# PaddlePaddle/MetaGym

Hardware: NVIDIA H100
Metric: env-steps/sec (quadrotor 6-DoF, 65k envs) (higher is better)
Workload: dtype f32

## Files before the change

metagym_b200/csrc/quad.cu:

```cuda
#include <math.h>
#include <stdlib.h>
#include <string.h>
#include <new>
#include <vector>

#include "mgb_common.cuh"
#include "quad_lanes.cuh"

namespace {

constexpr int kThreads = 64;
constexpr int kMaxObs = 19;

struct QuadConst {
    float h;
    float k1phi;
    float k1;
    float inv_phi;
    float hjm;
    float hk;
    float mm;
    float ct0, ct1, ct2;
    float vmin, vmax;
    float A[4], B[4];
    float px[4], py[4], pz[4];
    float Df[3], Dm[3];
    float cg[3];
    float hI[9];
    float gm;
    float c_hm;
    float c_h2m;
    float fail_r2, fail_v2, fail_w2;
    float dt, healthy, z_off;
    float init_v[3], init_w[3], noise_v, noise_w;
    int nt, task, substeps, obs_dim;
    int rk4_steps;
    float rk4_h;
    float inv_jm, inv_m;
    float Iinv[9];
    int simple;
};

struct QuadArgs {
    float4 *planes;
    int64_t n_pad;
    int64_t n;
    int64_t env_base;
    const float *act;
    float *obs;
    float *rew;
    uint8_t *done;
    int32_t *fail;
    float *final_obs;
    const float *targets;
    const int32_t *sat;
    int map_rows, map_cols, x_off, y_off;
    const int32_t *env2task;
    uint64_t seed;
    int auto_reset;
    int per_cta;
    int T;
    uint64_t act_seed;
    uint32_t t_base;
    float *act_out;
    MgbMirrors mir;
};

template <class T> struct VState {
    T p[3], v[3], om[3], w[4], R[9];
    int ct[Lanes<T>::N], ep[Lanes<T>::N];
};
using QState = VState<float>;

constexpr int kTileEnvs = 128;
constexpr int kPlanes = 6;

__device__ __forceinline__ float4 *tile_base(const QuadArgs &a, int64_t e)
{
    return a.planes + (e / kTileEnvs) * (kPlanes * kTileEnvs) + (e % kTileEnvs);
}

__device__ __forceinline__ void unpack_state(const float4 q[kPlanes], QState &s)
{
    s.p[0] = q[0].x; s.p[1] = q[0].y; s.p[2] = q[0].z; s.v[0] = q[0].w;
    s.v[1] = q[1].x; s.v[2] = q[1].y; s.om[0] = q[1].z; s.om[1] = q[1].w;
    s.om[2] = q[2].x; s.w[0] = q[2].y; s.w[1] = q[2].z; s.w[2] = q[2].w;
    s.w[3] = q[3].x; s.R[0] = q[3].y; s.R[1] = q[3].z; s.R[2] = q[3].w;
    s.R[3] = q[4].x; s.R[4] = q[4].y; s.R[5] = q[4].z; s.R[6] = q[4].w;
    s.R[7] = q[5].x; s.R[8] = q[5].y; s.ct[0] = __float_as_int(q[5].z); s.ep[0] = __float_as_int(q[5].w);
}
__device__ __forceinline__ void pack_state(const QState &s, float4 q[kPlanes])
{
    q[0] = make_float4(s.p[0], s.p[1], s.p[2], s.v[0]);
    q[1] = make_float4(s.v[1], s.v[2], s.om[0], s.om[1]);
    q[2] = make_float4(s.om[2], s.w[0], s.w[1], s.w[2]);
    q[3] = make_float4(s.w[3], s.R[0], s.R[1], s.R[2]);
    q[4] = make_float4(s.R[3], s.R[4], s.R[5], s.R[6]);
    q[5] = make_float4(s.R[7], s.R[8], __int_as_float(s.ct[0]), __int_as_float(s.ep[0]));
}

__device__ __forceinline__ void load_state(const QuadArgs &a, int64_t e, QState &s)
{
    const float4 *b = tile_base(a, e);
    float4 q[kPlanes];
#pragma unroll
    for (int k = 0; k < kPlanes; ++k) q[k] = b[k * kTileEnvs];
    unpack_state(q, s);
}

__device__ __forceinline__ void store_state(const QuadArgs &a, int64_t e, const QState &s)
{
    float4 *b = tile_base(a, e);
    float4 q[kPlanes];
    pack_state(s, q);
#pragma unroll
    for (int k = 0; k < kPlanes; ++k) b[k * kTileEnvs] = q[k];
}

template <class T> __device__ __forceinline__ void get_lane_state(const VState<T> &s, int h, QState &o);
template <class T> __device__ __forceinline__ void set_lane_state(VState<T> &s, int h, const QState &o);

__device__ __forceinline__ void load_state2(const QuadArgs &a, int64_t e, VState<f2> &s)
{
    QState s0, s1;
    load_state(a, e, s0);
    load_state(a, e + 1, s1);
    set_lane_state(s, 0, s0);
    set_lane_state(s, 1, s1);
}
__device__ __forceinline__ void store_state2(const QuadArgs &a, int64_t e, const VState<f2> &s)
{
    QState s0, s1;
    get_lane_state(s, 0, s0);
    get_lane_state(s, 1, s1);
    store_state(a, e, s0);
    store_state(a, e + 1, s1);
}

template <class T> __device__ __forceinline__ void get_lane_state(const VState<T> &s, int h, QState &o)
{
#pragma unroll
    for (int k = 0; k < 3; ++k) { o.p[k] = lane(s.p[k], h); o.v[k] = lane(s.v[k], h); o.om[k] = lane(s.om[k], h); }
#pragma unroll
    for (int k = 0; k < 4; ++k) o.w[k] = lane(s.w[k], h);
#pragma unroll
    for (int k = 0; k < 9; ++k) o.R[k] = lane(s.R[k], h);
    o.ct[0] = s.ct[h];
    o.ep[0] = s.ep[h];
}
template <class T> __device__ __forceinline__ void set_lane_state(VState<T> &s, int h, const QState &o)
{
#pragma unroll
    for (int k = 0; k < 3; ++k) { set_lane(s.p[k], h, o.p[k]); set_lane(s.v[k], h, o.v[k]); set_lane(s.om[k], h, o.om[k]); }
#pragma unroll
    for (int k = 0; k < 4; ++k) set_lane(s.w[k], h, o.w[k]);
#pragma unroll
    for (int k = 0; k < 9; ++k) set_lane(s.R[k], h, o.R[k]);
    s.ct[h] = o.ct[0];
    s.ep[h] = o.ep[0];
}

template <class T> __device__ __forceinline__ T dot3(T a0, T b0, T a1, T b1, T a2, T b2)
{
    return vfma(a2, b2, vfma(a1, b1, vmul(a0, b0)));
// ... 356 lines not shown
    for (int k = 0; k < 9; ++k) set_lane(s.R[k], h, (k % 4 == 0) ? 1.f : 0.f);
}

__device__ __forceinline__ void philox_reset_draws(uint64_t seed, int64_t genv, int ep, double u[12])
{
    const uint2 key = make_uint2((uint32_t)seed, (uint32_t)(seed >> 32));
#pragma unroll
    for (int j = 0; j < 3; ++j) {
        const uint4 r = mgb_philox4x32_10(
            make_uint4((uint32_t)genv, (uint32_t)((uint64_t)genv >> 32), (uint32_t)ep, MGB_STREAM_RESET + j), key);
        u[4 * j + 0] = (double)mgb_u01(r.x);
        u[4 * j + 1] = (double)mgb_u01(r.y);
        u[4 * j + 2] = (double)mgb_u01(r.z);
        u[4 * j + 3] = (double)mgb_u01(r.w);
    }
}

template <class T> struct TargetRows {
    T cur[3];
    T nxt[3];
};
template <class T>
__device__ __forceinline__ void prefetch_targets(const QuadConst &c, const float *trow, int ct, int h, TargetRows<T> &tr)
{
    const int t = ct < c.nt - 1 ? ct : c.nt - 1;
    const float *g = trow + 3 * (ct - 1), *q = trow + 3 * t;
    set_lane(tr.cur[0], h, __ldg(g)); set_lane(tr.cur[1], h, __ldg(g + 1)); set_lane(tr.cur[2], h, __ldg(g + 2));
    set_lane(tr.nxt[0], h, __ldg(q)); set_lane(tr.nxt[1], h, __ldg(q + 1)); set_lane(tr.nxt[2], h, __ldg(q + 2));
}

__device__ __forceinline__ int slice_bound(double v, int len)
{
    long long x = v < -2.0e9 ? -2000000000LL : (v > 2.0e9 ? 2000000000LL : (long long)v);
    if (x < 0) { x += len; if (x < 0) x = 0; }
    if (x > len) x = len;
    return (int)x;
}

__device__ __forceinline__ bool map_collision(const QuadArgs &a, float x_old, float y_old, float z_old, float x_new,
                                              float y_new, float z_new)
{
    const double xo = (double)x_old + a.x_off, xn = (double)x_new + a.x_off;
    const double yo = (double)y_old + a.y_off, yn = (double)y_new + a.y_off;
    const double x_min = floor(fmin(xo, xn)), x_max = ceil(fmax(xo, xn));
    const double y_min = floor(fmin(yo, yn)), y_max = ceil(fmax(yo, yn));
    const int z_lo = (int)floorf(fminf(z_old, z_new)), z_hi = (int)ceilf(fmaxf(z_old, z_new));
    const int ys = slice_bound(y_min, a.map_rows), ye = slice_bound(y_max + 1.0, a.map_rows);
    const int xs = slice_bound(x_min, a.map_cols), xe = slice_bound(x_max + 1.0, a.map_cols);
    int any = 0;
    if (ys < ye && xs < xe) {
        const int W = a.map_cols + 1;
        any = (a.sat[ye * W + xe] - a.sat[ys * W + xe] - a.sat[ye * W + xs] + a.sat[ys * W + xs]) > 0 ? 1 : 0;
    }
    return z_lo < any || z_hi < any;
}

template <class T>
__device__ __forceinline__ void observe_reset(const QuadConst &c, const QuadArgs &a, int64_t e, const VState<T> &s, int h,
                                              T *o)
{
    set_lane(o[0], h, lane(s.v[0], h)); set_lane(o[1], h, lane(s.v[1], h)); set_lane(o[2], h, lane(s.v[2], h));
    set_lane(o[3], h, 0.f); set_lane(o[4], h, 0.f); set_lane(o[5], h, 0.f);
    set_lane(o[6], h, 0.f * -9.8f); set_lane(o[7], h, 0.f * -9.8f); set_lane(o[8], h, -9.8f);
    set_lane(o[9], h, lane(s.om[0], h)); set_lane(o[10], h, lane(s.om[1], h)); set_lane(o[11], h, lane(s.om[2], h));
    set_lane(o[12], h, -0.f); set_lane(o[13], h, 0.f); set_lane(o[14], h, 0.f);
    set_lane(o[15], h, 0.f + c.z_off);
    if (c.task == MGB_TASK_VELOCITY_CONTROL) {
        const float *trow = a.targets + ((int64_t)a.env2task[e] * c.nt) * 3;
        const int t = s.ct[h] < c.nt - 1 ? s.ct[h] : c.nt - 1;
        set_lane(o[16], h, __ldg(trow + 3 * t)); set_lane(o[17], h, __ldg(trow + 3 * t + 1));
        set_lane(o[18], h, __ldg(trow + 3 * t + 2));
    }
}

template <class T>
__device__ __forceinline__ void finish_step(const QuadConst &c, const QuadArgs &a, int64_t e, VState<T> &s,
                                            const T adj[9], T id, T z_old, T x_old, T y_old, T power,
                                            const int fail[Lanes<T>::N], const TargetRows<T> &tr, T *o, T &reward,
                                            int done_flag[Lanes<T>::N], bool write_final[Lanes<T>::N])
{
    constexpr int N = Lanes<T>::N;
    T bv[3], Ri[9];
    observe(c, s, adj, id, o, bv, Ri);
    if (c.task == MGB_TASK_VELOCITY_CONTROL) {
        o[16] = tr.nxt[0]; o[17] = tr.nxt[1]; o[18] = tr.nxt[2];
    }
    reward = vneg(vmin(vmul(c.dt, power), bc<T>(c.healthy)));
    int done[N];
#pragma unroll
    for (int h = 0; h < N; ++h) done[h] = 0;
    if (c.task == MGB_TASK_VELOCITY_CONTROL) {
        const T g0 = tr.cur[0], g1 = tr.cur[1], g2 = tr.cur[2];
        T diff = bc<T>(0.f);
#pragma unroll
        for (int r = 0; r < 3; ++r) diff = vadd(diff, vabs(vsub(dot3(Ri[3 * r], g0, Ri[3 * r + 1], g1, Ri[3 * r + 2], g2), bv[r])));
        reward = vadd(reward, vmul(-0.001f, diff));
    } else {
        const T z_new = vadd(s.p[2], c.z_off);
        T bonus, vn, on;
        if (c.task == MGB_TASK_HOVERING_CONTROL) {
            vn = vsqrt(sq3(s.v));
            on = vsqrt(sq3(s.om));
        }
#pragma unroll
        for (int h = 0; h < N; ++h) {
            bool coll;
            if (a.sat) coll = map_collision(a, lane(x_old, h), lane(y_old, h), lane(z_old, h), lane(s.p[0], h),
                                            lane(s.p[1], h), lane(z_new, h));
            else coll = fminf(lane(z_old, h), lane(z_new, h)) < 0.f;
            float tr = coll ? 0.f : c.healthy;
            if (c.task == MGB_TASK_HOVERING_CONTROL) {
                tr -= lane(vn, h) + lane(on, h);
                const float zm = fabsf(0.f - lane(s.p[2], h));
                tr += zm < 0.5f ? 10.f : fmaxf(-20.f, 0.5f - zm);
            }
            set_lane(bonus, h, tr);
            if (coll) { done[h] = 1; s.ct[h] = 0; }
        }
        reward = vadd(reward, bonus);
    }
#pragma unroll
    for (int h = 0; h < N; ++h) {
        if (s.ct[h] == c.nt) { done[h] = 1; s.ct[h] = 0; }
        if (fail[h]) { done[h] = 1; s.ct[h] = 0; }
        done_flag[h] = done[h];
        write_final[h] = false;
        if (done[h] && a.auto_reset) {
            write_final[h] = true;
            s.ep[h] += 1;
            double u[12];
            philox_reset_draws(a.seed, a.env_base + e + h, s.ep[h], u);
            reset_env(c, s, h, u);
        }
    }
}

__device__ __forceinline__ void publish_tile(float *gobs, const float *tile, int64_t e0, int rows, int D)
{
    const uint32_t bytes = (uint32_t)rows * (uint32_t)D * 4u;
    float *dst = gobs + e0 * D;
    if ((bytes & 15u) == 0 && ((reinterpret_cast<uintptr_t>(dst) & 15u) == 0)) {
        mgb_fence_proxy_async();
        __syncthreads();
        if (threadIdx.x == 0) {
            mgb_bulk_store(dst, tile, bytes);
            mgb_bulk_commit();
        }
    } else {
        __syncthreads();
        for (int i = threadIdx.x; i < rows * D; i += blockDim.x) dst[i] = tile[i];
    }
}

__device__ __forceinline__ void publish_tile_mirrored(const MgbMirrors &m, float *gobs, const float *tile, int64_t e0,
                                                      int rows, int D)
{
    const uint32_t bytes = (uint32_t)rows * (uint32_t)D * 4u;
    float *dst = gobs + e0 * D;
    if ((bytes & 15u) == 0 && ((reinterpret_cast<uintptr_t>(dst) & 15u) == 0)) {
        mgb_fence_proxy_async();
        __syncthreads();
        if (threadIdx.x == 0) {
            mgb_bulk_store(dst, tile, bytes);
            mgb_mirror_bulk_store(m, dst, tile, bytes);
            mgb_bulk_commit();
        }
    } else {
        __syncthreads();
        for (int i = threadIdx.x; i < rows * D; i += blockDim.x) {
            dst[i] = tile[i];
            mgb_mirror_store(m, dst + i, tile[i]);
        }
    }
}

template <bool SIMPLE, bool EARLY, class T>
__device__ __forceinline__ void step_body(const QuadConst &c, const QuadArgs &a, int64_t e, int nact, VState<T> &s,
                                          const T V[4], float *trow, float *frow, int &final_mask)
{
    constexpr int N = Lanes<T>::N;
    const int D = c.obs_dim;
    T adj[9], id, power;
    adjugate(s.R, adj, id);
    TargetRows<T> tr;
    int ct_now[N];
#pragma unroll
    for (int h = 0; h < N; ++h) {
        s.ct[h] += 1;
        ct_now[h] = s.ct[h];
    }
    const bool vel = c.task == MGB_TASK_VELOCITY_CONTROL;
    if (EARLY && vel) {
#pragma unroll
        for (int h = 0; h < N; ++h) {
            const int64_t eh = h < nact ? e + h : e;
            prefetch_targets(c, a.targets + ((int64_t)__ldg(a.env2task + eh) * c.nt) * 3, ct_now[h], h, tr);
        }
    }
    const T z_old = vadd(s.p[2], c.z_off);
    const T x_old = s.p[0], y_old = s.p[1];
    int fail[N];
    if (N == 1 && c.rk4_steps > 0) {
        QState s1;
        get_lane_state(s, 0, s1);
        float adj1[9], id1, pw1;
        fail[0] = integrate_rk4<SIMPLE>(c, s1, make_float4(lane(V[0], 0), lane(V[1], 0), lane(V[2], 0), lane(V[3], 0)),
                                        adj1, id1, pw1);
        set_lane_state(s, 0, s1);
#pragma unroll
        for (int k = 0; k < 9; ++k) set_lane(adj[k], 0, adj1[k]);
        set_lane(id, 0, id1);
        set_lane(power, 0, pw1);
    } else {
        const bool failed = integrate<SIMPLE, T>(c, s, V, adj, id, power, fail);
        if (N > 1 && failed) {
#pragma unroll 1
            for (int h = 0; h < N; ++h) {
                QState s1;
                load_state(a, e + h, s1);
                float adj1[9], id1, pw1;
                adjugate(s1.R, adj1, id1);
                const float V1[4] = {lane(V[0], h), lane(V[1], h), lane(V[2], h), lane(V[3], h)};
                int f1[1];
                integrate<SIMPLE, float>(c, s1, V1, adj1, id1, pw1, f1);
                s1.ct[0] = s.ct[h];
                s1.ep[0] = s.ep[h];
                set_lane_state(s, h, s1);
#pragma unroll
                for (int k = 0; k < 9; ++k) set_lane(adj[k], h, adj1[k]);
                set_lane(id, h, id1);
                set_lane(power, h, pw1);
                fail[h] = f1[0];
            }
        }
    }
    if (!EARLY && vel) {
#pragma unroll
        for (int h = 0; h < N; ++h) {
            const int64_t eh = h < nact ? e + h : e;
            prefetch_targets(c, a.targets + ((int64_t)__ldg(a.env2task + eh) * c.nt) * 3, ct_now[h], h, tr);
        }
    }
    const bool state_first = N == 1 && !EARLY && vel;
    if (state_first) {
        QState s1;
        get_lane_state(s, 0, s1);
        if (s1.ct[0] == c.nt || fail[0]) s1.ct[0] = 0;
        store_state(a, e, s1);
    }
    T o[kMaxObs], reward;
    int done[N];
    bool wf[N];
    finish_step(c, a, e, s, adj, id, z_old, x_old, y_old, power, fail, tr, o, reward, done, wf);
    bool stored = false;
    if constexpr (N == 2) {
        if (nact == 2) {
            store_state2(a, e, s);
            *reinterpret_cast<float2 *>(a.rew + e) = reward.v;
            *reinterpret_cast<uchar2 *>(a.done + e) = make_uchar2((uint8_t)done[0], (uint8_t)done[1]);
            if (a.fail) *reinterpret_cast<int2 *>(a.fail + e) = make_int2(fail[0], fail[1]);
            stored = true;
        }
    }
    if (!stored) {
#pragma unroll
        for (int h = 0; h < N; ++h) {
            if (h < nact) {
                QState s1;
                get_lane_state(s, h, s1);
                if (!state_first || wf[h]) store_state(a, e + h, s1);
                a.rew[e + h] = lane(reward, h);
                a.done[e + h] = (uint8_t)done[h];
                if (a.fail) a.fail[e + h] = fail[h];
            }
        }
    }
#pragma unroll
    for (int h = 0; h < N; ++h) {
        if (h < nact) {
            float *tr_h = trow + h * D;
            if (wf[h]) {
                if (a.final_obs) {
                    float *fr_h = frow + h * D;
#pragma unroll
                    for (int k = 0; k < 16; ++k) fr_h[k] = lane(o[k], h);
                    if (D == 19) { fr_h[16] = lane(o[16], h); fr_h[17] = lane(o[17], h); fr_h[18] = lane(o[18], h); }
                    final_mask |= 1 << h;
                }
                observe_reset(c, a, e + h, s, h, o);
            }
#pragma unroll
            for (int k = 0; k < 16; ++k) tr_h[k] = lane(o[k], h);
            if (D == 19) { tr_h[16] = lane(o[16], h); tr_h[17] = lane(o[17], h); tr_h[18] = lane(o[18], h); }
        }
    }
}

__device__ __forceinline__ void publish_final(const QuadArgs &a, const float *ftile, int64_t e, int local_row, int lanes,
                                              int final_mask, int D)
{
    if (!a.final_obs) return;
    if (__syncthreads_or(final_mask)) {
        for (int h = 0; h < lanes; ++h) {
            if (final_mask & (1 << h)) {
                float *dst = a.final_obs + (e + h) * D;
                const float *frow = ftile + (local_row + h) * D;
                for (int k = 0; k < D; ++k) dst[k] = frow[k];
            }
        }
    }
}

template <bool SIMPLE>
__global__ void __launch_bounds__(kThreads) quad_step_kernel(const __grid_constant__ QuadConst c,
                                                             const __grid_constant__ QuadArgs a)
{
    __shared__ __align__(128) float tile[kThreads * kMaxObs];
    __shared__ __align__(128) float ftile[kThreads * kMaxObs];
    const int64_t e0 = (int64_t)blockIdx.x * kThreads;
    const int64_t e = e0 + threadIdx.x;
    const int rows = (int)((a.n - e0) < kThreads ? (a.n - e0) : kThreads);
    const int D = c.obs_dim;
    const bool active = e < a.n;
    int final_mask = 0;

    asm volatile("griddepcontrol.launch_dependents;");
    asm volatile("griddepcontrol.wait;" ::: "memory");

    if (active) {
        QState s;
        load_state(a, e, s);
        const float4 act = __ldg(reinterpret_cast<const float4 *>(a.act) + e);
        const float V[4] = {act.x, act.y, act.z, act.w};
        step_body<SIMPLE, false, float>(c, a, e, 1, s, V, tile + threadIdx.x * D, ftile + threadIdx.x * D, final_mask);
    }
    publish_tile(a.obs, tile, e0, rows, D);
    publish_final(a, ftile, e, threadIdx.x, 1, final_mask, D);
    if (threadIdx.x == 0) mgb_bulk_wait_read<0>();
}

template <bool SIMPLE>
__global__ void __launch_bounds__(512, 1) quad_step_wide_kernel(const __grid_constant__ QuadConst c,
                                                                const __grid_constant__ QuadArgs a)
{
    extern __shared__ __align__(128) float wide_smem[];
    const int per = a.per_cta;
    float *tile = wide_smem, *ftile = wide_smem + (size_t)per * kMaxObs;
    const int64_t e0 = (int64_t)blockIdx.x * per;
    const int64_t e = e0 + threadIdx.x;
    int rows = (int)((a.n - e0) < per ? (a.n - e0) : per);
    if (rows < 0) rows = 0;
    const int D = c.obs_dim;
    const bool active = (int)threadIdx.x < rows;
    int final_mask = 0;
    asm volatile("griddepcontrol.launch_dependents;");
    asm volatile("griddepcontrol.wait;" ::: "memory");
    if (active) {
        QState s;
        load_state(a, e, s);
        const float4 act = __ldg(reinterpret_cast<const float4 *>(a.act) + e);
        const float V[4] = {act.x, act.y, act.z, act.w};
        step_body<SIMPLE, true, float>(c, a, e, 1, s, V, tile + threadIdx.x * D, ftile + threadIdx.x * D, final_mask);
    }
    if (rows > 0) publish_tile(a.obs, tile, e0, rows, D);
    else __syncthreads();
    publish_final(a, ftile, e, threadIdx.x, 1, final_mask, D);
    if (threadIdx.x == 0) mgb_bulk_wait_read<0>();
}

template <bool SIMPLE>
__global__ void __launch_bounds__(256, 1) quad_step2_kernel(const __grid_constant__ QuadConst c,
                                                            const __grid_constant__ QuadArgs a)
{
    extern __shared__ __align__(128) float pair_smem[];
    const int per = a.per_cta;
    float *tile = pair_smem, *ftile = pair_smem + (size_t)per * kMaxObs;
    const int64_t e0 = (int64_t)blockIdx.x * per;
    int rows = (int)((a.n - e0) < per ? (a.n - e0) : per);
    if (rows < 0) rows = 0;
    const int le = 2 * (int)threadIdx.x;
    const int64_t e = e0 + le;
    const int D = c.obs_dim;
    const int nact = rows - le >= 2 ? 2 : (rows - le > 0 ? 1 : 0);
    int final_mask = 0;
    asm volatile("griddepcontrol.launch_dependents;");
    asm volatile("griddepcontrol.wait;" ::: "memory");
    if (nact > 0) {
        VState<f2> s;
        load_state2(a, e, s);
        const float4 a0 = __ldg(reinterpret_cast<const float4 *>(a.act) + e);
        const float4 a1 = nact == 2 ? __ldg(reinterpret_cast<const float4 *>(a.act) + e + 1) : make_float4(0.f, 0.f, 0.f, 0.f);
        const f2 V[4] = {pack2(a0.x, a1.x), pack2(a0.y, a1.y), pack2(a0.z, a1.z), pack2(a0.w, a1.w)};
        step_body<SIMPLE, true, f2>(c, a, e, nact, s, V, tile + le * D, ftile + le * D, final_mask);
    }
    if (rows > 0) publish_tile(a.obs, tile, e0, rows, D);
    else __syncthreads();
    publish_final(a, ftile, e, le, 2, final_mask, D);
    if (threadIdx.x == 0) mgb_bulk_wait_read<0>();
}

constexpr int kStreamThreads = 128;

template <bool SIMPLE>
__global__ void __launch_bounds__(kStreamThreads, 4) quad_stream_kernel(const __grid_constant__ QuadConst c,
                                                                        const __grid_constant__ QuadArgs a)
{
    __shared__ __align__(128) float4 stage[2][7][kStreamThreads];
    __shared__ __align__(128) float tile[kStreamThreads * kMaxObs];
    __shared__ __align__(128) float ftile[kStreamThreads * kMaxObs];
    __shared__ __align__(8) uint64_t full[2];
    const int D = c.obs_dim;
    const int64_t n_tiles = (a.n + kStreamThreads - 1) / kStreamThreads;
    const int tid = threadIdx.x;

    asm volatile("griddepcontrol.launch_dependents;");
    asm volatile("griddepcontrol.wait;" ::: "memory");
    if (tid == 0) {
        mgb_mbar_init(&full[0], 1);
        mgb_mbar_init(&full[1], 1);
        mgb_fence_mbar_init();
    }
    __syncthreads();

    auto fetch = [&](int64_t t, int st) {
        const int64_t e0 = t * kStreamThreads;
        const uint32_t rows = (uint32_t)((a.n - e0) < kStreamThreads ? (a.n - e0) : kStreamThreads);
        static_assert(kStreamThreads == kTileEnvs, "one CTA iteration = one state tile");
        mgb_mbar_expect_tx(&full[st], 6u * kTileEnvs * 16u + rows * 16u);
        mgb_bulk_load(stage[st][0], a.planes + t * (6 * kTileEnvs), 6u * kTileEnvs * 16u, &full[st]);
        mgb_bulk_load(stage[st][6], reinterpret_cast<const float4 *>(a.act) + e0, rows * 16u, &full[st]);
    };

    int64_t t = blockIdx.x;
    if (tid == 0 && t < n_tiles) fetch(t, 0);
    uint32_t phase[2] = {0u, 0u};
    int st = 0;
    for (; t < n_tiles; t += gridDim.x, st ^= 1) {
        const int64_t t_next = t + gridDim.x;
        if (tid == 0 && t_next < n_tiles) fetch(t_next, st ^ 1);
        mgb_mbar_wait(&full[st], phase[st]);
        phase[st] ^= 1u;
        const int64_t e0 = t * kStreamThreads, e = e0 + tid;
        const int rows = (int)((a.n - e0) < kStreamThreads ? (a.n - e0) : kStreamThreads);
        int final_mask = 0;
        if (tid == 0) mgb_bulk_wait_read<0>();
        __syncthreads();
        if (tid < rows) {
            QState s;
            float4 q[kPlanes];
#pragma unroll
            for (int k = 0; k < kPlanes; ++k) q[k] = stage[st][k][tid];
            unpack_state(q, s);
            const float4 act = stage[st][6][tid];
            const float V[4] = {act.x, act.y, act.z, act.w};
            step_body<SIMPLE, true, float>(c, a, e, 1, s, V, tile + tid * D, ftile + tid * D, final_mask);
        }
        publish_tile(a.obs, tile, e0, rows, D);
        publish_final(a, ftile, e, tid, 1, final_mask, D);
        __syncthreads();
    }
    if (tid == 0) mgb_bulk_wait_read<0>();
}

template <bool SIMPLE, int XM>
__global__ void __launch_bounds__(kThreads, 8) quad_rollout_kernel(const __grid_constant__ QuadConst c,
                                                                const __grid_constant__ QuadArgs a)
{
    __shared__ __align__(128) float tiles[2][kThreads * kMaxObs];
    const int64_t e0 = (int64_t)blockIdx.x * kThreads;
    const int64_t e = e0 + threadIdx.x;
    const int rows = (int)((a.n - e0) < kThreads ? (a.n - e0) : kThreads);
    const int D = c.obs_dim;
    const bool active = e < a.n;
    QState s;
    float adj[9], id = 1.f;
    if (active) {
        load_state(a, e, s);
        adjugate(s.R, adj, id);
    }
    const uint2 akey = make_uint2((uint32_t)a.act_seed, (uint32_t)(a.act_seed >> 32));
    const int64_t genv = a.env_base + e;
    const float *trow = nullptr;
    if (active && c.task == MGB_TASK_VELOCITY_CONTROL) trow = a.targets + ((int64_t)__ldg(a.env2task + e) * c.nt) * 3;
    float4 act_next = make_float4(0.f, 0.f, 0.f, 0.f);
    if (active && a.act) act_next = __ldg(reinterpret_cast<const float4 *>(a.act) + e);
    for (int t = 0; t < a.T; ++t) {
        float *tile = tiles[t & 1];
        if (threadIdx.x == 0) mgb_bulk_wait_read<1>();
        __syncthreads();
        uint32_t done_byte = 0;
        if (active) {
// ... 343 lines not shown

extern "C" int mgb_quad_set_options(mgb_quad *h, int auto_reset, uint64_t seed)
{
    MGB_REQUIRE(h, "null handle");
    h->auto_reset = auto_reset ? 1 : 0;
    h->seed = seed;
    return MGB_OK;
}

extern "C" int mgb_quad_set_map(mgb_quad *h, const int32_t *map_host, int32_t rows, int32_t cols)
{
    MGB_REQUIRE(h, "null handle");
    MgbDeviceGuard guard(h->device);
    MGB_CUDA(cudaDeviceSynchronize());
    cudaFree(h->sat);
    h->sat = nullptr;
    h->map_rows = h->map_cols = h->x_off = h->y_off = 0;
    if (!map_host) return MGB_OK;
    MGB_REQUIRE(h->c.task != MGB_TASK_VELOCITY_CONTROL, "velocity_control has no map (env.py:101-104)");
    MGB_REQUIRE(rows > 0 && cols > 0 && rows <= 8192 && cols <= 8192, "map size out of range");
    int starts = 0, sr = 0, sc = 0;
    for (int r = 0; r < rows; ++r)
        for (int q = 0; q < cols; ++q)
            if (map_host[(size_t)r * cols + q] == -1) { ++starts; sr = r; sc = q; }
    MGB_REQUIRE(starts == 1, "the map must mark exactly one start cell with -1 (env.py:108-109)");
    std::vector<int32_t> sat((size_t)(rows + 1) * (cols + 1), 0);
    for (int r = 0; r < rows; ++r)
        for (int q = 0; q < cols; ++q) {
            const int v = (r == sr && q == sc) ? 0 : map_host[(size_t)r * cols + q];
            sat[(size_t)(r + 1) * (cols + 1) + q + 1] = (v != 0 ? 1 : 0) + sat[(size_t)r * (cols + 1) + q + 1] +
                                                        sat[(size_t)(r + 1) * (cols + 1) + q] - sat[(size_t)r * (cols + 1) + q];
        }
    MGB_CUDA(cudaMalloc(&h->sat, sat.size() * sizeof(int32_t)));
    MGB_CUDA(cudaMemcpy(h->sat, sat.data(), sat.size() * sizeof(int32_t), cudaMemcpyHostToDevice));
    h->map_rows = rows; h->map_cols = cols; h->x_off = sc; h->y_off = sr;
    return MGB_OK;
}

extern "C" int mgb_quad_set_targets(mgb_quad *h, const float *tbl_dev, int32_t n_tasks, const int32_t *env2task_dev)
{
    MGB_REQUIRE(h && tbl_dev && env2task_dev, "null argument");
    MGB_REQUIRE(n_tasks > 0, "n_tasks must be positive");
    MgbDeviceGuard guard(h->device);
    MGB_CUDA(cudaDeviceSynchronize());
    cudaFree(h->targets); h->targets = nullptr;
    cudaFree(h->env2task); h->env2task = nullptr;
    const size_t tb = sizeof(float) * 3 * (size_t)h->c.nt * (size_t)n_tasks;
    MGB_CUDA(cudaMalloc(&h->targets, tb));
    MGB_CUDA(cudaMalloc(&h->env2task, sizeof(int32_t) * h->n));
    MGB_CUDA(cudaMemcpy(h->targets, tbl_dev, tb, cudaMemcpyDeviceToDevice));
    MGB_CUDA(cudaMemcpy(h->env2task, env2task_dev, sizeof(int32_t) * h->n, cudaMemcpyDeviceToDevice));
    MGB_CUDA(cudaDeviceSynchronize());
    h->n_tasks = n_tasks;
    return MGB_OK;
}

static int check_ready(const mgb_quad *h)
{
    if (h->c.task == MGB_TASK_VELOCITY_CONTROL && !h->targets) {
        mgb_set_error("velocity_control: call mgb_quad_set_targets before reset/step");
        return MGB_ERR_STATE;
    }
    return MGB_OK;
}

extern "C" int mgb_quad_make_targets(mgb_quad *h, const float *act_dev, int32_t n_tasks, float *tbl_dev, void *stream)
{
    MgbRange nvtx_range("mgb_quad_make_targets");
    MGB_REQUIRE(h && act_dev && tbl_dev, "null argument");
    MGB_REQUIRE(n_tasks > 0, "n_tasks must be positive");
    MgbDeviceGuard guard(h->device);
    cudaStream_t st = (cudaStream_t)stream;
    const int threads = 32, blocks = (n_tasks + threads - 1) / threads;
    if (h->c.simple) quad_targets_kernel<true><<<blocks, threads, 0, st>>>(h->c, act_dev, n_tasks, tbl_dev);
    else quad_targets_kernel<false><<<blocks, threads, 0, st>>>(h->c, act_dev, n_tasks, tbl_dev);
    MGB_CUDA(cudaGetLastError());
    h->launches += 1;
    return MGB_OK;
}

extern "C" int mgb_quad_reset(mgb_quad *h, const uint8_t *mask_dev, const double *noise_dev, float *obs_dev,
                              void *stream)
{
    MgbRange nvtx_range("mgb_quad_reset");
    MGB_REQUIRE(h, "null handle");
    int rc = check_ready(h);
    if (rc) return rc;
    MgbDeviceGuard guard(h->device);
    QuadArgs a = base_args(h);
    a.obs = obs_dev;
    quad_reset_kernel<<<(unsigned)((h->n + kThreads - 1) / kThreads), kThreads, 0, (cudaStream_t)stream>>>(
        h->c, a, mask_dev, noise_dev);
    MGB_CUDA(cudaGetLastError());
    h->launches += 1;
    return MGB_OK;
}

enum StepKernel { STEP_TILE = 0, STEP_WIDE = 1, STEP_STREAM = 2, STEP_PACKED = 3 };

static StepKernel choose_step_kernel(const mgb_quad *h, const QuadArgs &a)
{
    const unsigned blocks = (unsigned)((a.n + kThreads - 1) / kThreads);
    const bool act16 = (reinterpret_cast<uintptr_t>(a.act) & 15u) == 0;
    if (h->stream_kernel && (int64_t)blocks > (int64_t)h->num_sms * 32 && act16) return STEP_STREAM;
    if (h->packed && h->c.rk4_steps == 0 && a.n >= 2) {
        const bool aligned = act16 && (reinterpret_cast<uintptr_t>(a.rew) & 7u) == 0 &&
                             (reinterpret_cast<uintptr_t>(a.done) & 1u) == 0 && (reinterpret_cast<uintptr_t>(a.fail) & 7u) == 0;
        if (aligned) return STEP_PACKED;
    }
    const bool single_wave = a.n <= (int64_t)h->num_sms * 512 && a.n >= (int64_t)h->num_sms * 64;
    const int64_t wide_max = (int64_t)h->num_sms * (h->wide_kernel > 0 ? 512 : 384);
    if (h->wide_kernel != 0 && single_wave && a.n <= wide_max) return STEP_WIDE;
    return STEP_TILE;
}

static int launch_step(mgb_quad *h, const QuadArgs &a, cudaStream_t st)
{
    const unsigned blocks = (unsigned)((a.n + kThreads - 1) / kThreads);
    cudaLaunchConfig_t cfg;
    memset(&cfg, 0, sizeof(cfg));
    cfg.gridDim = dim3(blocks);
    cfg.blockDim = dim3(kThreads);
    cfg.stream = st;
    cudaLaunchAttribute attr[1];
    attr[0].id = cudaLaunchAttributeProgrammaticStreamSerialization;
    attr[0].val.programmaticStreamSerializationAllowed = h->pdl ? 1 : 0;
    cfg.attrs = attr;
    cfg.numAttrs = 1;
    const StepKernel which = choose_step_kernel(h, a);
    if (which == STEP_STREAM) {
        cfg.gridDim = dim3((unsigned)(h->num_sms * 4));
        cfg.blockDim = dim3(kStreamThreads);
        if (h->c.simple) MGB_CUDA(cudaLaunchKernelEx(&cfg, quad_stream_kernel<true>, h->c, a));
        else MGB_CUDA(cudaLaunchKernelEx(&cfg, quad_stream_kernel<false>, h->c, a));
    } else if (which == STEP_WIDE || which == STEP_PACKED) {
        const int lanes = which == STEP_PACKED ? 2 : 1;
        int per;
        if (a.n <= (int64_t)h->num_sms * 512 && a.n >= (int64_t)h->num_sms * 64) per = (int)((a.n + h->num_sms - 1) / h->num_sms);
        else per = a.n < (int64_t)h->num_sms * 64 ? 64 : 256;
        per = (per + 3) / 4 * 4;
        QuadArgs aw = a;
        aw.per_cta = per;
        cfg.gridDim = dim3((unsigned)((a.n + per - 1) / per));
        cfg.blockDim = dim3((unsigned)((per / lanes + 31) / 32 * 32));
        cfg.dynamicSmemBytes = (size_t)per * kMaxObs * 4 * 2;
        if (which == STEP_PACKED) {
            if (h->c.simple) MGB_CUDA(cudaLaunchKernelEx(&cfg, quad_step2_kernel<true>, h->c, aw));
            else MGB_CUDA(cudaLaunchKernelEx(&cfg, quad_step2_kernel<false>, h->c, aw));
        } else {
            if (h->c.simple) MGB_CUDA(cudaLaunchKernelEx(&cfg, quad_step_wide_kernel<true>, h->c, aw));
            else MGB_CUDA(cudaLaunchKernelEx(&cfg, quad_step_wide_kernel<false>, h->c, aw));
        }
    } else {
        if (h->c.simple) MGB_CUDA(cudaLaunchKernelEx(&cfg, quad_step_kernel<true>, h->c, a));
        else MGB_CUDA(cudaLaunchKernelEx(&cfg, quad_step_kernel<false>, h->c, a));
    }
    MGB_CUDA(cudaGetLastError());
    h->launches += 1;
    return MGB_OK;
}

extern "C" const char *mgb_quad_step_kernel(const mgb_quad *h)
{
    if (!h) return "";
    QuadArgs a = base_args(h);
    switch (choose_step_kernel(h, a)) {
    case STEP_STREAM: return h->c.simple ? "quad_stream_kernel<true>" : "quad_stream_kernel<false>";
    case STEP_PACKED: return h->c.simple ? "quad_step2_kernel<true>" : "quad_step2_kernel<false>";
    case STEP_WIDE: return h->c.simple ? "quad_step_wide_kernel<true>" : "quad_step_wide_kernel<false>";
    default: return h->c.simple ? "quad_step_kernel<true>" : "quad_step_kernel<false>";
    }
}

extern "C" int mgb_quad_step(mgb_quad *h, const float *act_dev, float *obs_dev, float *rew_dev, uint8_t *done_dev,
                             int32_t *fail_dev, float *final_obs_dev, void *stream)
{
    MgbRange nvtx_range("mgb_quad_step");
    MGB_REQUIRE(h && act_dev && obs_dev && rew_dev && done_dev, "null argument");
    MGB_REQUIRE((reinterpret_cast<uintptr_t>(act_dev) & 15u) == 0, "act_dev must be 16-byte aligned");
    int rc = check_ready(h);
    if (rc) return rc;
    MgbDeviceGuard guard(h->device);
    QuadArgs a = base_args(h);
    a.act = act_dev; a.obs = obs_dev; a.rew = rew_dev; a.done = done_dev; a.fail = fail_dev;
    a.final_obs = final_obs_dev;
    return launch_step(h, a, (cudaStream_t)stream);
}

extern "C" int mgb_quad_rollout(mgb_quad *h, int32_t T, const float *act_dev, uint64_t act_seed, float *act_out_dev,
                                float *obs_dev, float *rew_dev, uint8_t *done_dev, void *stream)
{
    MgbRange nvtx_range("mgb_quad_rollout");
    MGB_REQUIRE(h, "null handle");
    MGB_REQUIRE(T > 0, "T must be positive");
    MGB_REQUIRE((reinterpret_cast<uintptr_t>(act_dev) & 15u) == 0, "act_dev must be 16-byte aligned");
    int rc = check_ready(h);
    if (rc) return rc;
    MgbDeviceGuard guard(h->device);
    QuadArgs a = base_args(h);
    a.act = act_dev; a.obs = obs_dev; a.rew = rew_dev; a.done = done_dev;
    a.T = T; a.act_seed = act_seed; a.t_base = h->t_base; a.act_out = act_out_dev;
    const unsigned blocks = (unsigned)((a.n + kThreads - 1) / kThreads);
    a.mir = h->mir;
    if (h->mir.count != 0)
        MGB_REQUIRE(h->mir_win.holds(obs_dev, (uint64_t)T * h->n * h->c.obs_dim * 4) &&
                        h->mir_win.holds(rew_dev, (uint64_t)T * h->n * 4) && h->mir_win.holds(done_dev, (uint64_t)T * h->n) &&
                        h->mir_win.holds(act_out_dev, (uint64_t)T * h->n * 16),
                    "mirrors are on but an output lies outside the mirrored arena (set_mirrors([]) first)");
    if (h->mir.count == MGB_MIRROR_MULTICAST) {
        MGB_REQUIRE(h->n % 4 == 0, "multicast outputs need num_envs % 4 == 0");
        MGB_REQUIRE((((uintptr_t)done_dev | (uintptr_t)rew_dev | (uintptr_t)obs_dev) & 3) == 0 && ((uintptr_t)act_out_dev & 15) == 0,
                    "multicast outputs must be 4-byte (actions: 16-byte) aligned");
        if (h->c.simple) quad_rollout_kernel<true, 2><<<blocks, kThreads, 0, (cudaStream_t)stream>>>(h->c, a);
        else quad_rollout_kernel<false, 2><<<blocks, kThreads, 0, (cudaStream_t)stream>>>(h->c, a);
    } else if (h->mir.count > 0) {
        if (h->c.simple) quad_rollout_kernel<true, 1><<<blocks, kThreads, 0, (cudaStream_t)stream>>>(h->c, a);
        else quad_rollout_kernel<false, 1><<<blocks, kThreads, 0, (cudaStream_t)stream>>>(h->c, a);
    } else {
        if (h->c.simple) quad_rollout_kernel<true, 0><<<blocks, kThreads, 0, (cudaStream_t)stream>>>(h->c, a);
        else quad_rollout_kernel<false, 0><<<blocks, kThreads, 0, (cudaStream_t)stream>>>(h->c, a);
    }
    MGB_CUDA(cudaGetLastError());
    h->t_base += (uint32_t)T;
    h->launches += 1;
    return MGB_OK;
}

extern "C" int mgb_quad_set_mirrors(mgb_quad *h, int count, const int64_t *byte_delta)
{
    MGB_REQUIRE(h, "null handle");
    MGB_REQUIRE(count >= 0 && count <= MGB_MAX_MIRRORS && (count == 0 || byte_delta), "count out of range");
    MgbMirrors m = {};
    for (int i = 0; i < count; ++i) {
        MGB_REQUIRE((byte_delta[i] & 15) == 0, "mirror deltas must be multiples of 16 bytes");
        m.delta[i] = byte_delta[i];
    }
    m.count = count;
    h->mir = m;
    return MGB_OK;
}

extern "C" int mgb_quad_set_mirror_window(mgb_quad *h, const void *base, uint64_t bytes)
{
    MGB_REQUIRE(h, "null handle");
    h->mir_win.base = reinterpret_cast<uintptr_t>(base);
    h->mir_win.bytes = bytes;
    return MGB_OK;
}

extern "C" int mgb_quad_set_multicast(mgb_quad *h, int64_t byte_delta)
{
    MGB_REQUIRE(h, "null handle");
    MGB_REQUIRE((byte_delta & 15) == 0, "multicast delta must be a multiple of 16 bytes");
    MgbMirrors m = {};
    if (byte_delta != 0) { m.count = MGB_MIRROR_MULTICAST; m.delta[0] = byte_delta; }
    h->mir = m;
    return MGB_OK;
}

static int ensure_host_staging(mgb_quad *h)
{
    if (h->d_act) return MGB_OK;
    const size_t n = (size_t)h->n, D = (size_t)h->c.obs_dim;
    MGB_CUDA(cudaMalloc(&h->d_act, n * 16));
    MGB_CUDA(cudaMalloc(&h->d_obs, n * D * 4));
    MGB_CUDA(cudaMalloc(&h->d_rew, n * 4));
    MGB_CUDA(cudaMalloc(&h->d_done, n));
    MGB_CUDA(cudaMalloc(&h->d_fail, n * 4));
    MGB_CUDA(cudaMalloc(&h->d_final, n * D * 4));
    MGB_CUDA(cudaMemset(h->d_fail, 0, n * 4));
    MGB_CUDA(cudaMemset(h->d_final, 0, n * D * 4));
    MGB_CUDA(cudaMallocHost(&h->h_act, n * 16));
    MGB_CUDA(cudaMallocHost(&h->h_obs, n * D * 4));
    MGB_CUDA(cudaMallocHost(&h->h_rew, n * 4));
    MGB_CUDA(cudaMallocHost(&h->h_done, n));
    MGB_CUDA(cudaMallocHost(&h->h_fail, n * 4));
    MGB_CUDA(cudaMallocHost(&h->h_final, n * D * 4));
    return MGB_OK;
}

static void *pinned_device_alias(const void *p)
{
    cudaPointerAttributes at;
    if (cudaPointerGetAttributes(&at, p) != cudaSuccess) { cudaGetLastError(); return nullptr; }
    if (at.type != cudaMemoryTypeHost) return nullptr;
    return at.devicePointer;
}

extern "C" int mgb_quad_step_host(mgb_quad *h, const float *act_host, float *obs_host, float *rew_host,
                                  uint8_t *done_host, int32_t *fail_host, float *final_obs_host, void *stream)
{
    MgbRange nvtx_range("mgb_quad_step_host");
    MGB_REQUIRE(h && act_host && obs_host && rew_host && done_host, "null argument");
    int rc = check_ready(h);
    if (rc) return rc;
    MgbDeviceGuard guard(h->device);
    rc = ensure_host_staging(h);
    if (rc) return rc;
    const size_t n = (size_t)h->n, D = (size_t)h->c.obs_dim;
    cudaStream_t st = (cudaStream_t)stream;
    void *da = pinned_device_alias(act_host), *dob = pinned_device_alias(obs_host), *dr = pinned_device_alias(rew_host),
         *dd = pinned_device_alias(done_host);
    void *df = fail_host ? pinned_device_alias(fail_host) : nullptr;
    void *dfo = final_obs_host ? pinned_device_alias(final_obs_host) : nullptr;
    const bool opt_ok = (!fail_host || df) && (!final_obs_host || dfo);
    if (h->zerocopy && da && dob && dr && dd && opt_ok && (reinterpret_cast<uintptr_t>(da) & 15u) == 0) {
        QuadArgs a = base_args(h);
        a.act = (const float *)da; a.obs = (float *)dob; a.rew = (float *)dr; a.done = (uint8_t *)dd;
// ... 53 lines not shown
```

Before: 8.279 billion.

## Stagger warp cohorts in 256-thread step kernel with named barriers and per-warp stores

Adds a 256-thread variant of the per-env step kernel, used when the env count falls between one and two CTAs' worth of envs per SM. The first half of the warps signals a named barrier after its state stores, and the second half waits on it before starting. This staggers the load and compute phases of the two halves. Observation tiles are now published per warp with bulk stores, and final obs are written per thread, which removes the CTA-wide __syncthreads in the publish path. The stagger delays half the CTA and adds more bulk-store transactions in exchange.

```diff
diff --git a/metagym_b200/csrc/quad.cu b/metagym_b200/csrc/quad.cu
--- a/metagym_b200/csrc/quad.cu
+++ b/metagym_b200/csrc/quad.cu
@@ -10,6 +10,7 @@
 namespace {
 
 constexpr int kThreads = 64;
+constexpr int kCohortThreads = 256;
 constexpr int kMaxObs = 19;
 
 struct QuadConst {
@@ -672,6 +673,24 @@
     }
 }
 
+__device__ __forceinline__ void publish_warp_rows(float *gobs, const float *wtile, int64_t w0, int rows, int D)
+{
+    const int lane = threadIdx.x % 32;
+    float *dst = gobs + w0 * D;
+    if (rows >= 32 && (reinterpret_cast<uintptr_t>(dst) & 15u) == 0) {
+        mgb_fence_proxy_async();
+        __syncwarp();
+        if (lane == 0) {
+            mgb_bulk_store(dst, wtile, 32u * (uint32_t)D * 4u);
+            mgb_bulk_commit();
+        }
+    } else {
+        __syncwarp();
+        const int m = rows < 32 ? rows : 32;
+        for (int i = lane; i < m * D; i += 32) dst[i] = wtile[i];
+    }
+}
+
 __device__ __forceinline__ void publish_tile_mirrored(const MgbMirrors &m, float *gobs, const float *tile, int64_t e0,
                                                       int rows, int D)
 {
@@ -696,7 +715,7 @@
 
 template <bool SIMPLE, bool EARLY, class T>
 __device__ __forceinline__ void step_body(const QuadConst &c, const QuadArgs &a, int64_t e, int nact, VState<T> &s,
-                                          const T V[4], float *trow, float *frow, int &final_mask)
+                                          const T V[4], float *trow, float *frow, int &final_mask, bool gate = false)
 {
     constexpr int N = Lanes<T>::N;
     const int D = c.obs_dim;
@@ -768,6 +787,10 @@
         if (s1.ct[0] == c.nt || fail[0]) s1.ct[0] = 0;
         store_state(a, e, s1);
     }
+    if (gate) {
+        __syncwarp();
+        asm volatile("bar.arrive 1, 256;" ::: "memory");
+    }
     T o[kMaxObs], reward;
     int done[N];
     bool wf[N];
@@ -831,17 +854,21 @@
     }
 }
 
-template <bool SIMPLE>
-__global__ void __launch_bounds__(kThreads) quad_step_kernel(const __grid_constant__ QuadConst c,
-                                                             const __grid_constant__ QuadArgs a)
-{
-    __shared__ __align__(128) float tile[kThreads * kMaxObs];
-    __shared__ __align__(128) float ftile[kThreads * kMaxObs];
-    const int64_t e0 = (int64_t)blockIdx.x * kThreads;
+template <bool SIMPLE, bool COHORTS>
+__global__ void __launch_bounds__(COHORTS ? kCohortThreads : kThreads, COHORTS ? 2 : 0)
+    quad_step_kernel(const __grid_constant__ QuadConst c, const __grid_constant__ QuadArgs a)
+{
+    constexpr int kCta = COHORTS ? kCohortThreads : kThreads;
+    __shared__ __align__(128) float tile[kCta * kMaxObs];
+    __shared__ __align__(128) float ftile[kCta * kMaxObs];
+    const int64_t e0 = (int64_t)blockIdx.x * kCta;
     const int64_t e = e0 + threadIdx.x;
-    const int rows = (int)((a.n - e0) < kThreads ? (a.n - e0) : kThreads);
+    const int rows = (int)((a.n - e0) < kCta ? (a.n - e0) : kCta);
     const int D = c.obs_dim;
     const bool active = e < a.n;
+    const int warp = threadIdx.x / 32;
+    const bool cohort_a = COHORTS && rows == kCta && warp < kCta / 64;
+    const bool cohort_b = COHORTS && rows == kCta && warp >= kCta / 64;
     int final_mask = 0;
 
     asm volatile("griddepcontrol.launch_dependents;");
@@ -852,11 +879,21 @@
         load_state(a, e, s);
         const float4 act = __ldg(reinterpret_cast<const float4 *>(a.act) + e);
         const float V[4] = {act.x, act.y, act.z, act.w};
-        step_body<SIMPLE, false, float>(c, a, e, 1, s, V, tile + threadIdx.x * D, ftile + threadIdx.x * D, final_mask);
-    }
-    publish_tile(a.obs, tile, e0, rows, D);
-    publish_final(a, ftile, e, threadIdx.x, 1, final_mask, D);
-    if (threadIdx.x == 0) mgb_bulk_wait_read<0>();
+        if (cohort_b) asm volatile("bar.sync 1, 256;" ::: "memory");
+        step_body<SIMPLE, false, float>(c, a, e, 1, s, V, tile + threadIdx.x * D, ftile + threadIdx.x * D, final_mask,
+                                        cohort_a);
+    }
+    if constexpr (COHORTS) {
+        publish_warp_rows(a.obs, tile + warp * 32 * D, e0 + warp * 32, rows - warp * 32, D);
+        if (a.final_obs && final_mask) {
+            for (int k = 0; k < D; ++k) a.final_obs[e * D + k] = ftile[threadIdx.x * D + k];
+        }
+        if (threadIdx.x % 32 == 0) mgb_bulk_wait_read<0>();
+    } else {
+        publish_tile(a.obs, tile, e0, rows, D);
+        publish_final(a, ftile, e, threadIdx.x, 1, final_mask, D);
+        if (threadIdx.x == 0) mgb_bulk_wait_read<0>();
+    }
 }
 
 template <bool SIMPLE>
@@ -1506,8 +1543,15 @@
             else MGB_CUDA(cudaLaunchKernelEx(&cfg, quad_step_wide_kernel<false>, h->c, aw));
         }
     } else {
-        if (h->c.simple) MGB_CUDA(cudaLaunchKernelEx(&cfg, quad_step_kernel<true>, h->c, a));
-        else MGB_CUDA(cudaLaunchKernelEx(&cfg, quad_step_kernel<false>, h->c, a));
+        if (a.n >= (int64_t)h->num_sms * kCohortThreads && a.n <= (int64_t)h->num_sms * 2 * kCohortThreads) {
+            cfg.gridDim = dim3((unsigned)((a.n + kCohortThreads - 1) / kCohortThreads));
+            cfg.blockDim = dim3(kCohortThreads);
+            if (h->c.simple) MGB_CUDA(cudaLaunchKernelEx(&cfg, quad_step_kernel<true, true>, h->c, a));
+            else MGB_CUDA(cudaLaunchKernelEx(&cfg, quad_step_kernel<false, true>, h->c, a));
+        } else {
+            if (h->c.simple) MGB_CUDA(cudaLaunchKernelEx(&cfg, quad_step_kernel<true, false>, h->c, a));
+            else MGB_CUDA(cudaLaunchKernelEx(&cfg, quad_step_kernel<false, false>, h->c, a));
+        }
     }
     MGB_CUDA(cudaGetLastError());
     h->launches += 1;
```

After: 8.616 billion, median of 6. 4.1% higher.
